# odecaux/DSP-Bench

Measured on AMD Instinct MI355X. Metric: Msamples/s offline render+8192-pt FFT, 48kHz stereo, 1/2/4/8 GPU; %HBM roofline, higher is better.
Workload: dtype f32

## Files before the change

dsp-bench_amd/csrc/stft_pk.hpp:

```cpp
#pragma once
#include "fft_pk.hpp"
#include "frame_load.hpp"

namespace dspb {

enum { kPkNoBarDft = 1, kPkNoBarTw = 2, kPkNoBarSplit = 4, kPkRenderCached = 8, kPkNtMag = 16, kPkMagLds = 32,
       kPkOldSplit = 64, kPkAbNoRender = 128, kPkAbNoMag = 256, kPkMagStage = 512, kPkOcc3 = 1024,
       kPkMemAos = 2048, kPkNoRemap = 4096, kPkAbNoXpose = 8192, kPkMemPf = 16384, kPkW1 = 65536,
       kPkMemHop = 131072, kPkNoReuse = 262144 };
constexpr int kPkDefaultOpt = kPkNoBarDft | kPkNoBarTw | kPkNoBarSplit;
constexpr int kPkPerOpt = kPkDefaultOpt | kPkW1;

typedef float f4u __attribute__((ext_vector_type(4), aligned(4)));
typedef float f4a __attribute__((ext_vector_type(4)));

template <bool NT, typename T>
__device__ __forceinline__ void st(T *p, T v) {
    if constexpr (NT) __builtin_nontemporal_store(v, p);
    else *p = v;
}

template <bool NT>
__device__ __forceinline__ void st4u(float *p, f4u v) {
    if constexpr (NT) __builtin_nontemporal_store(v, reinterpret_cast<f4u *>(p));
    else *reinterpret_cast<f4u *>(p) = v;
}

template <int KM>
__device__ __forceinline__ void put_bin(float *mrow, uint32_t K, uint32_t k, float m) {
    if constexpr (KM == kKPartial) {
        if (k < K) mrow[k] = m;
    } else {
        mrow[k] = m;
        if constexpr (KM == kKMirror) mrow[(8192u - k) & 8191u] = m;
    }
}

constexpr int kPkRowRegs = 66;
template <int KM, bool BAR, bool NOSTORE = false, bool STAGE = false, bool STAGE_NT = false, bool KEEP = false>
__device__ __forceinline__ void split_y2(const cx2 (&Y2)[32], float *mrow, uint32_t K, const v2f *tw,
                                         uint32_t lane, float *lds, float *M = nullptr) {
    static_assert(!STAGE || KM == kKHalf, "staged rows: 4097 bins");
    static_assert(!KEEP || (KM == kKHalf && !NOSTORE && !STAGE), "kept rows: 4097 bins, the dword row stores");
    float acc = 0.f;
    const uint32_t a = (uint32_t)(reinterpret_cast<uintptr_t>(mrow) >> 2) & 3u;
    float *sl = lds + a;
    const uint32_t src = ((64u - lane) & 63u) * 4u;
    const bool l0 = lane == 0;
    const v2f wl = tw[lane];
#pragma unroll
    for (int q = 0; q < 16; ++q) {
        if (BAR) __builtin_amdgcn_sched_barrier(0);
        const cx2 a = Y2[q == 0 ? 0 : 32 - q], b = Y2[31 - q];
        const float sxr = l0 ? (q == 0 ? a.r.x : a.r.y) : b.r.y;
        const float sxi = l0 ? (q == 0 ? a.i.x : a.i.y) : b.i.y;
        const float syr = l0 ? (q == 0 ? a.r.y : a.r.x) : b.r.x;
        const float syi = l0 ? (q == 0 ? a.i.y : a.i.x) : b.i.x;
        const cx2 Pp = cx2{v2f{bperm(src, sxr), bperm(src, syr)}, v2f{bperm(src, sxi), bperm(src, syi)}};
        const cx2 Z = Y2[q];
        const cx2 E = cx2{Z.r + Pp.r, Z.i - Pp.i};
        const cx2 D = cx2{Z.r - Pp.r, Z.i + Pp.i};
        v2f u = wl;
        if (q) u = v2f{wl.x, wl.x} * v2f{kW128_re[q], kW128_im[q]} + v2f{wl.y, wl.y} * v2f{-kW128_im[q], kW128_re[q]};
        v2f rU2, iU2;
        asm("v_pk_mul_f32 %0, %1, %2 op_sel:[0,1] op_sel_hi:[1,0] neg_hi:[0,1]" : "=v"(rU2) : "v"(D.r), "v"(u));
        asm("v_pk_mul_f32 %0, %1, %2 op_sel:[0,1] op_sel_hi:[1,0] neg_hi:[0,1]" : "=v"(iU2) : "v"(D.i), "v"(u));
        const cx2 T = cx2{D.i * u + rU2, iU2 - D.r * u};
        const cx2 X1 = E + T;
        const cx2 X2 = E - T;
        const v2f q1 = X1.r * X1.r + X1.i * X1.i;
        const v2f q2 = X2.r * X2.r + X2.i * X2.i;
        const uint32_t k = lane + 64u * (uint32_t)q;
        if constexpr (KEEP) {
            (M + lane)[64 * (4 * q)] = __builtin_amdgcn_sqrtf(q1.x);
            (M + lane)[64 * (4 * q + 1)] = __builtin_amdgcn_sqrtf(q1.y);
            (M + lane)[64 * (4 * q + 2)] = __builtin_amdgcn_sqrtf(q2.x);
            (M + lane)[64 * (4 * q + 3)] = __builtin_amdgcn_sqrtf(q2.y);
        } else if constexpr (NOSTORE) {
            acc += __builtin_amdgcn_sqrtf(q1.x) + __builtin_amdgcn_sqrtf(q1.y) + __builtin_amdgcn_sqrtf(q2.x) +
                   __builtin_amdgcn_sqrtf(q2.y);
        } else if constexpr (STAGE) {
            (sl + lane)[64 * q] = __builtin_amdgcn_sqrtf(q1.x);
            (sl + 2048u + lane)[64 * q] = __builtin_amdgcn_sqrtf(q1.y);
            (sl + 4096u - lane)[-64 * q] = __builtin_amdgcn_sqrtf(q2.x);
            (sl + 2048u - lane)[-64 * q] = __builtin_amdgcn_sqrtf(q2.y);
        } else if constexpr (KM == kKHalf) {
            st<STAGE_NT>(&(mrow + lane)[64 * q], __builtin_amdgcn_sqrtf(q1.x));
            st<STAGE_NT>(&(mrow + 2048u + lane)[64 * q], __builtin_amdgcn_sqrtf(q1.y));
            st<STAGE_NT>(&(mrow + 4096u - lane)[-64 * q], __builtin_amdgcn_sqrtf(q2.x));
            st<STAGE_NT>(&(mrow + 2048u - lane)[-64 * q], __builtin_amdgcn_sqrtf(q2.y));
        } else {
            put_bin<KM>(mrow, K, k, __builtin_amdgcn_sqrtf(q1.x));
            put_bin<KM>(mrow, K, 2048u + k, __builtin_amdgcn_sqrtf(q1.y));
            put_bin<KM>(mrow, K, 4096u - k, __builtin_amdgcn_sqrtf(q2.x));
            put_bin<KM>(mrow, K, 2048u - k, __builtin_amdgcn_sqrtf(q2.y));
        }
    }
    if constexpr (NOSTORE) {
        if (acc == -1.f) mrow[lane] = acc;
        return;
    }
    if (l0) {
        const cx z1 = cx{Y2[16].r.x, Y2[16].i.x}, z2 = cx{Y2[16].r.y, Y2[16].i.y};
        const cx E = cx{z1.r + z2.r, z1.i - z2.i}, D = cx{z1.r - z2.r, z1.i + z2.i};
        const float c = 0x1.6a09e6p-1f;
        const cx T = cx{c * (D.i - D.r), -c * (D.i + D.r)};
        const cx X1 = E + T, X2 = E - T;
        const float m1 = __builtin_amdgcn_sqrtf(__builtin_fmaf(X1.r, X1.r, X1.i * X1.i));
        const float m2 = __builtin_amdgcn_sqrtf(__builtin_fmaf(X2.r, X2.r, X2.i * X2.i));
        if constexpr (KEEP) {
            M[4096] = m1;
            M[4097] = m2;
        } else if constexpr (STAGE) {
            sl[1024] = m1;
            sl[3072] = m2;
        } else {
            put_bin<KM>(mrow, K, 1024u, m1);
            put_bin<KM>(mrow, K, 3072u, m2);
        }
    }
    if constexpr (STAGE) {
        lds_fence();
        const uint32_t j0 = a ? 1u : 0u, j1 = (4093u + a) >> 2;
        float *gb = mrow - a;
#pragma unroll
        for (int it = 0; it < 16; ++it) {
            const uint32_t j = j0 + 64u * (uint32_t)it + lane;
            if (it < 15 || j <= j1)
            {
                const float4 q = reinterpret_cast<const float4 *>(lds)[j];
                st<STAGE_NT>(reinterpret_cast<f4a *>(gb + 4u * j), f4a{q.x, q.y, q.z, q.w});
            }
        }
        const uint32_t head = 4u * j0 - a, tail0 = 4u * j1 + 4u - a;
        if (lane < head) mrow[lane] = sl[lane];
        if (lane >= 8u && tail0 + (lane - 8u) < 4097u) mrow[tail0 + lane - 8u] = sl[tail0 + lane - 8u];
    }
}

template <bool NT>
__device__ __forceinline__ void store_row_y2(const float (&M)[kPkRowRegs], float *mrow, uint32_t lane) {
#pragma unroll
    for (int q = 0; q < 16; ++q) {
        st<NT>(&(mrow + lane)[64 * q], M[4 * q]);
        st<NT>(&(mrow + 2048u + lane)[64 * q], M[4 * q + 1]);
        st<NT>(&(mrow + 4096u - lane)[-64 * q], M[4 * q + 2]);
        st<NT>(&(mrow + 2048u - lane)[-64 * q], M[4 * q + 3]);
    }
    if (lane == 0) {
        mrow[1024] = M[64];
        mrow[3072] = M[65];
    }
}

template <int OPT>
constexpr uint32_t pk_waves_per_block() { return (OPT & kPkW1) ? 1u : 4u; }
constexpr uint32_t kPkWpb = pk_waves_per_block<kPkDefaultOpt>();
constexpr uint32_t kPkPerWpb = pk_waves_per_block<kPkPerOpt>();

template <int PER>
__device__ __forceinline__ void per_gather(const Stft8kArgs &A, uint32_t p0, cx2 (&X)[PER >= 2 ? PER / 2 : 1]) {
    constexpr int NJ = PER >= 2 ? PER / 2 : 1;
    const float *T = A.map.table;
    if (A.map.closed) {
#pragma unroll
        for (int jj = 0; jj < NJ; ++jj) {
            const uint32_t q0 = (p0 + 256u * jj) & A.map.b_mask;
            const uint32_t q1 = (p0 + 256u * jj + (PER >= 2 ? 128u : 0u)) & A.map.b_mask;
            X[jj] = cx2{v2f{ramp_value(A.map, q0), ramp_value(A.map, q1)},
                        v2f{ramp_value(A.map, q0 + 1), ramp_value(A.map, q1 + 1)}};
        }
    } else {
#pragma unroll
        for (int jj = 0; jj < NJ; ++jj) {
            const uint32_t q0 = (p0 + 256u * jj) & A.map.b_mask;
            const uint32_t q1 = (p0 + 256u * jj + (PER >= 2 ? 128u : 0u)) & A.map.b_mask;
            X[jj] = cx2{v2f{T[q0], T[q1]}, v2f{T[q0 + 1], T[q1 + 1]}};
        }
    }
}

template <int PER, bool NT>
__device__ __forceinline__ void per_render_hop(const Stft8kArgs &A, float *o, uint32_t lane,
                                               const cx2 (&X)[PER >= 2 ? PER / 2 : 1]) {
    constexpr int NS = PER >= 2 ? PER : 1;
    v2f st[NS];
#pragma unroll
    for (int b = 0; b < NS; ++b) st[b] = v2f{X[b / 2].r[b & 1], X[b / 2].i[b & 1]};
    if (A.H == 4096u) {
#pragma unroll
        for (int b = 0; b < 32; ++b)
            dspb::st<NT>(reinterpret_cast<v2f *>(o + 128u * (uint32_t)b) + lane, st[b % NS]);
    } else {
#pragma unroll
        for (int b = 0; b < 64; ++b)
            if (128u * (uint32_t)b < A.H)
                dspb::st<NT>(reinterpret_cast<v2f *>(o + 128u * (uint32_t)b) + lane, st[b % NS]);
    }
}

template <int SRC, int KM, MapKind MK, bool POW2, bool WINC, int PER = 0, int OPT = kPkDefaultOpt, int OCC = 2>
__global__ __launch_bounds__(64 * pk_waves_per_block<OPT>()) __attribute__((amdgpu_waves_per_eu(OCC, OCC)))
void stft8192_pk_kernel(Stft8kArgs A) {
    constexpr uint32_t WPB = pk_waves_per_block<OPT>();
    __shared__ __attribute__((aligned(16))) float lds_all[WPB][OCC >= 3 ? 64 * 33 : 64 * 65];
    const uint32_t lane = threadIdx.x & 63u;
    const uint32_t wave = __builtin_amdgcn_readfirstlane(threadIdx.x >> 6);
    const uint32_t ch = blockIdx.y;
    uint64_t f = (uint64_t)((OPT & kPkNoRemap) ? blockIdx.x : xcd_remap(blockIdx.x, gridDim.x)) * WPB + wave;
    constexpr bool SOA = WINC && MK == MapKind::Ramp && PER > 0 && SRC == kSrcRender;
    constexpr bool REUSE = SOA && KM == kKHalf && OCC == 2 &&
                           !(OPT & (kPkNoReuse | kPkOldSplit | kPkMagLds | kPkMagStage | kPkAbNoRender | kPkAbNoMag | kPkAbNoXpose));
    uint32_t nrun = 1;
    if constexpr (REUSE) {
        if (A.run > 1u) {
            if (f < A.run_waves) {
                f *= A.run;
                const uint64_t left = A.F - f;
                nrun = left < A.run ? (uint32_t)left : A.run;
            } else {
                f = A.F + (f - A.run_waves);
            }
        }
    }
    constexpr bool MSOA = WINC && SRC == kSrcMemory && !(OPT & kPkMemAos);
    constexpr bool W4 = SOA && (8 % (PER >= 2 ? PER / 2 : 1)) == 0 && OCC == 2 &&
                        !(OPT & (kPkOldSplit | kPkMagLds | kPkAbNoXpose));
    const uint64_t fs = f * (uint64_t)A.H;
    if (f >= A.F) {
        if constexpr (SOA) {
            if (fs < A.tail_end) {
                const uint32_t p0 = (uint32_t)(A.goff + fs) + 2u * lane;
                float *o = A.out.p[ch] + fs;
                const uint64_t n = A.tail_end - fs;
#pragma unroll 4
                for (uint32_t b = 0; 128u * b < A.H; ++b) {
                    const uint32_t e = 128u * b + 2u * lane;
                    if (e < n) {
                        const uint32_t q = (p0 + 128u * b) & A.map.b_mask;
                        const v2f t = A.map.closed ? v2f{ramp_value(A.map, q), ramp_value(A.map, q + 1)}
                                                   : v2f{A.map.table[q], A.map.table[q + 1]};
                        reinterpret_cast<v2f *>(o + 128u * b)[lane] = t;
                    }
                }
            }
        }
        return;
    }
    float *lds = lds_all[wave];
    const float *x = (ch < A.in_ch) ? A.in.p[ch] : nullptr;

    static_assert(OCC == 2 || (SOA && !(OPT & (kPkOldSplit | kPkMagLds | kPkMagStage))),
                  "3 waves per SIMD: the PER path with split_y2");
    cx tlo[8];
    cx2 thp[4];
    if constexpr (OCC == 2) {
#pragma unroll
        for (int j = 1; j < 8; ++j) {
            const v2f a = (A.tw + 8192u + 64u * (uint32_t)(j - 1))[lane];
            tlo[j] = cx{a.x, a.y};
        }
        const float4 *tp4 = reinterpret_cast<const float4 *>(A.tw + 8192u + 896u);
#pragma unroll
        for (int h = 0; h < 4; ++h) {
            const float4 t = tp4[64u * (uint32_t)h + lane];
            thp[h] = cx2{v2f{t.x, t.y}, v2f{t.z, t.w}};
        }
    }
    float4 wbase = float4{0.f, 0.f, 0.f, 0.f};
    if constexpr (WINC) wbase = A.wbase[lane];

    cx2 P[32];
    if constexpr (SOA || MSOA) {
        constexpr int NJ = PER >= 2 ? PER / 2 : 1;
        cx2 X[NJ];
        if constexpr (SOA) {
            per_gather<PER>(A, (uint32_t)(A.goff + fs) + 2u * lane, X);
            if (!(OPT & kPkAbNoRender) && nrun == 1u)
                per_render_hop<PER, !(OPT & kPkRenderCached)>(A, A.out.p[ch] + fs, lane, X);
        }
        const float ue = A.wb * wbase.x, ve = A.wb * wbase.y, uo = A.wb * wbase.z, vo = A.wb * wbase.w;
        if constexpr (SOA) {
            cx2 XA[NJ], XU[NJ], XV[NJ];
            const float wa = W4 ? 4.f * A.wa : A.wa;
#pragma unroll
            for (int jj = 0; jj < NJ; ++jj) {
                XA[jj] = cx2{X[jj].r * v2f{wa, wa}, X[jj].i * v2f{wa, wa}};
                XU[jj] = cx2{X[jj].r * v2f{ue, ue}, X[jj].i * v2f{uo, uo}};
                XV[jj] = cx2{X[jj].r * v2f{ve, ve}, X[jj].i * v2f{vo, vo}};
            }
            auto fma2 = [](v2f a, v2f b, v2f c) { return __builtin_elementwise_fma(a, b, c); };
            if constexpr (W4) {
                auto Sv = [](int j) { return v2f{kWinB_s[2 * j], kWinB_s[2 * j + 1]}; };
                auto Cv = [](int j) { return v2f{kWinB_c[2 * j], kWinB_c[2 * j + 1]}; };
#pragma unroll
                for (int j0 = 0; j0 < 8; ++j0) {
                    const int jj = j0 % NJ;
                    const v2f s0 = Sv(j0), s1 = Sv(j0 + 8), s2 = Sv(j0 + 16), s3 = Sv(j0 + 24);
                    const v2f c0 = Cv(j0), c1 = Cv(j0 + 8), c2 = Cv(j0 + 16), c3 = Cv(j0 + 24);
                    const cx2 xa = XA[jj], xu = XU[jj], xv = XV[jj];
                    const v2f sA = (s0 + s1) + (s2 + s3), cA = (c0 + c1) + (c2 + c3);
                    P[j0] = cx2{fma2(-xu.r, cA, fma2(xv.r, sA, xa.r)), fma2(-xu.i, cA, fma2(xv.i, sA, xa.i))};
                    const v2f sC = (s0 - s1) + (s2 - s3), cC = (c0 - c1) + (c2 - c3);
                    P[j0 + 16] = cx2{fma2(-xu.r, cC, xv.r * sC), fma2(-xu.i, cC, xv.i * sC)};
                    const v2f sT = s0 - s2, cT = c0 - c2, sQ = s1 - s3, cQ = c1 - c3;
                    const cx2 t1 = cx2{fma2(-xu.r, cT, xv.r * sT), fma2(-xu.i, cT, xv.i * sT)};
                    const cx2 q = cx2{fma2(-xu.r, cQ, xv.r * sQ), fma2(-xu.i, cQ, xv.i * sQ)};
                    P[j0 + 8] = cx2{t1.r + q.i, t1.i - q.r};
                    P[j0 + 24] = cx2{t1.r - q.i, t1.i + q.r};
                }
            } else {
#pragma unroll
                for (int j = 0; j < 32; ++j) {
                    const v2f C = v2f{kWinB_c[2 * j], kWinB_c[2 * j + 1]}, S = v2f{kWinB_s[2 * j], kWinB_s[2 * j + 1]};
                    const int jj = j % NJ;
                    P[j] = cx2{fma2(-XU[jj].r, C, fma2(XV[jj].r, S, XA[jj].r)),
                               fma2(-XU[jj].i, C, fma2(XV[jj].i, S, XA[jj].i))};
                }
            }
        } else {
#pragma unroll
        for (int j = 0; j < 32; ++j) {
            const v2f C = v2f{kWinB_c[2 * j], kWinB_c[2 * j + 1]}, S = v2f{kWinB_s[2 * j], kWinB_s[2 * j + 1]};
            const v2f we = (v2f{ve, ve} * S + v2f{A.wa, A.wa}) - v2f{ue, ue} * C;
            const v2f wo = (v2f{vo, vo} * S + v2f{A.wa, A.wa}) - v2f{uo, uo} * C;
            const v2f a = reinterpret_cast<const v2f *>(x + fs + 256u * (uint32_t)j)[lane];
            const v2f b = reinterpret_cast<const v2f *>(x + fs + 256u * (uint32_t)j + 128u)[lane];
            const cx2 xj = cx2{v2f{a.x, b.x}, v2f{a.y, b.y}};
            P[j] = cx2{xj.r * we, xj.i * wo};
        }
        }
    } else {
    cx v[64];
    if constexpr (SRC == kSrcMemory) {
        if (A.valid >= 8192u) {
#pragma unroll
            for (int b = 0; b < 64; ++b) {
                const v2f t = reinterpret_cast<const v2f *>(x + fs + 128u * (uint32_t)b)[lane];
                v[b] = cx{t.x, t.y};
            }
        } else {
#pragma unroll
            for (int b = 0; b < 64; ++b) {
                const uint32_t s = 2u * lane + 128u * (uint32_t)b;
                v2f t = v2f{0.f, 0.f};
                if (s < A.valid) t = reinterpret_cast<const v2f *>(x + fs + 128u * (uint32_t)b)[lane];
                v[b] = cx{t.x, t.y};
            }
        }
    } else {
        if constexpr (MK == MapKind::Ramp && POW2) {
            if (A.map.B >= 4u && A.map.B <= 4096u) lds_table_frame(A, lds, fs, lane, v);
            else s_render_frame<MK, POW2>(A, x, fs, lane, v);
        } else if constexpr (MK == MapKind::GainTable && POW2) {
            if (A.map.B >= 4u && A.map.B <= 512u) reg_gain_table_frame(A, x, fs, lane, v, ch);
            else if (A.map.B >= 4u && A.map.B <= 4096u) lds_gain_table_frame(A, lds, x, fs, lane, v, ch);
            else s_render_frame<MK, POW2>(A, x, fs, lane, v, ch);
        } else {
            s_render_frame<MK, POW2>(A, x, fs, lane, v, ch);
        }
        float *o = A.out.p[ch] + fs;
        constexpr bool NT = !(OPT & kPkRenderCached);
        if (A.H == 4096u) {
#pragma unroll
            for (int b = 0; b < 32; ++b)
                st<NT>(reinterpret_cast<v2f *>(o + 128u * (uint32_t)b) + lane, v2f{v[b].r, v[b].i});
        } else {
#pragma unroll
            for (int b = 0; b < 64; ++b)
                if (128u * (uint32_t)b < A.H)
                    st<NT>(reinterpret_cast<v2f *>(o + 128u * (uint32_t)b) + lane, v2f{v[b].r, v[b].i});
        }
    }

    {
        const v2f uu = v2f{A.wb * wbase.x, A.wb * wbase.z}, vv = v2f{A.wb * wbase.y, A.wb * wbase.w};
#pragma unroll
        for (int j = 0; j < 32; ++j) {
            v2f w[2];
#pragma unroll
            for (int h = 0; h < 2; ++h) {
                const int b = 2 * j + h;
                if constexpr (WINC) {
                    w[h] = (vv * kWinB_s[b] + v2f{A.wa, A.wa}) - uu * kWinB_c[b];
                } else {
                    w[h] = (A.win2 + 64u * (uint32_t)b)[lane];
                }
            }
            P[j] = cx2{v2f{v[2 * j].r * w[0].x, v[2 * j + 1].r * w[1].x},
                       v2f{v[2 * j].i * w[0].y, v[2 * j + 1].i * w[1].y}};
        }
    }
    }

    if constexpr (!(OPT & (kPkOldSplit | kPkMagLds))) {
        cx2 Y2[32];
        if constexpr (OCC >= 3) fft4096_pk_y2_lo<!(OPT & kPkNoBarDft)>(P, lds, A.tw, lane, Y2);
        else fft4096_pk_y2<!(OPT & kPkNoBarDft), !(OPT & kPkNoBarTw), (OPT & kPkAbNoXpose) != 0, NoHook, W4>(
            P, lds, tlo, thp, lane, Y2);
        if constexpr (REUSE) {
            if (nrun > 1u) {
                static_assert(64 * 65 >= 4098, "the kept row fits the wave's LDS tile");
                split_y2<KM, !(OPT & kPkNoBarSplit), false, false, false, true>(Y2, nullptr, A.K, A.tw, lane, lds, lds);
                float M[kPkRowRegs];
#pragma unroll
                for (int j = 0; j < 64; ++j) M[j] = (lds + lane)[64 * j];
                M[64] = lds[4096];
                M[65] = lds[4097];
                cx2 X[PER >= 2 ? PER / 2 : 1];
                per_gather<PER>(A, (uint32_t)(A.goff + fs) + 2u * lane, X);
                float *o = A.out.p[ch] + fs;
                float *mrow = A.mag.p[ch] + f * A.ld;
                for (uint32_t r = 0; r < nrun; ++r, o += A.H, mrow += A.ld) {
                    per_render_hop<PER, !(OPT & kPkRenderCached)>(A, o, lane, X);
                    store_row_y2<(OPT & kPkNtMag) != 0>(M, mrow, lane);
                }
                return;
            }
        }
        split_y2<KM, !(OPT & kPkNoBarSplit), (OPT & kPkAbNoMag) != 0, KM == kKHalf && (OPT & kPkMagStage) != 0,
                 (OPT & kPkNtMag) != 0>(Y2, A.mag.p[ch] + f * A.ld, A.K, A.tw, lane, lds);
        return;
    }

    cx zp[32], zm[32];
    fft4096_pk<false, !(OPT & kPkNoBarDft), !(OPT & kPkNoBarTw)>(P, lds, tlo, thp, lane, zp, zm);

    float *mrow = A.mag.p[ch] + f * A.ld;
    const uint32_t src = ((64u - lane) & 63u) * 4u;
    const bool l0 = lane == 0;
    const v2f wl2 = A.tw[lane];
    const cx wl = cx{wl2.x, wl2.y};
#pragma unroll
    for (int ka = 0; ka < 16; ++ka) {
        if (!(OPT & kPkNoBarSplit)) __builtin_amdgcn_sched_barrier(0);
        const cx a0 = ka == 0 ? zp[0] : zm[32 - ka], b0 = zm[31 - ka];
        const cx a1 = zm[16 - ka], b1 = zm[15 - ka];
        const cx s0 = cx{l0 ? a0.r : b0.r, l0 ? a0.i : b0.i};
        const cx s1 = cx{l0 ? a1.r : b1.r, l0 ? a1.i : b1.i};
        const cx2 Pp = cx2{v2f{bperm(src, s0.r), bperm(src, s1.r)}, v2f{bperm(src, s0.i), bperm(src, s1.i)}};
        const cx2 Z = cx2{v2f{zp[ka].r, zp[ka + 16].r}, v2f{zp[ka].i, zp[ka + 16].i}};
        const cx2 E = cx2{Z.r + Pp.r, Z.i - Pp.i};
        const cx2 D = cx2{Z.r - Pp.r, Z.i + Pp.i};
        const cx2 tw = cmulb(wl, cx2{v2f{kW128_re[ka], kW128_re[ka + 16]},
                                     v2f{kW128_im[ka], kW128_im[ka + 16]}});
        const cx2 T = cmul2(negi(D), tw);
        const cx2 X1 = E + T;
        const cx2 X2 = E - T;
        const v2f q1 = X1.r * X1.r + X1.i * X1.i;
        const v2f q2 = X2.r * X2.r + X2.i * X2.i;
        const float m1[2] = {__builtin_amdgcn_sqrtf(q1.x), __builtin_amdgcn_sqrtf(q1.y)};
        const float m2[2] = {__builtin_amdgcn_sqrtf(q2.x), __builtin_amdgcn_sqrtf(q2.y)};
#pragma unroll
        for (int h = 0; h < 2; ++h) {
            const uint32_t kk = (uint32_t)(ka + 16 * h);
            const uint32_t k1 = lane + 64u * kk;
            const uint32_t k2 = 4096u - k1;
            if constexpr (KM == kKHalf && (OPT & kPkMagLds)) {
                lds[64u * kk + lane] = m1[h];
                lds[4096u - 64u * kk - lane] = m2[h];
            } else if constexpr (KM == kKPartial) {
                if (k1 < A.K) mrow[k1] = m1[h];
                if (k2 < A.K) mrow[k2] = m2[h];
            } else {
                st<(OPT & kPkNtMag) != 0>(mrow + 64u * kk + lane, m1[h]);
                st<(OPT & kPkNtMag) != 0>(mrow + 4096u - 64u * kk - lane, m2[h]);
                if constexpr (KM == kKMirror) {
                    mrow[k1 == 0 ? 0u : 8192u - k1] = m1[h];
                    (mrow + 4096u + 64u * kk)[lane] = m2[h];
                }
            }
        }
    }
    if constexpr (KM == kKHalf && (OPT & kPkMagLds)) {
        if (l0) {
            const cx Z = zm[0];
            lds[2048] = 2.f * __builtin_amdgcn_sqrtf(__builtin_fmaf(Z.r, Z.r, Z.i * Z.i));
        }
        lds_fence();
#pragma unroll
        for (int i = 0; i < 16; ++i) {
            const float4 q = reinterpret_cast<const float4 *>(lds)[64 * i + lane];
            st4u<(OPT & kPkNtMag) != 0>(mrow + 256u * (uint32_t)i + 4u * lane, f4u{q.x, q.y, q.z, q.w});
        }
        if (l0) mrow[4096] = lds[4096];
        return;
    }
    if (l0) {
        const cx Z = zm[0];
        const float m = 2.f * __builtin_amdgcn_sqrtf(__builtin_fmaf(Z.r, Z.r, Z.i * Z.i));
        if (KM != kKPartial || 2048u < A.K) mrow[2048] = m;
        if (KM == kKMirror) mrow[6144] = m;
    }
}

int launch_pk_paths(const Stft8kArgs &A, bool fused, int km, bool pow2, bool winc, dim3 grid, hipStream_t s);
bool stft_pk_ab_dispatch(const Stft8kArgs &A, uint32_t C, bool fused, int opt, dim3 grid, hipStream_t s, int *st);


}
```

Baseline: 670,300.

## Stage reused magnitude rows through LDS for aligned vector stores and render early

When a run of identical frames reuses one magnitude row, each row is now written to LDS, read back as aligned float4s and stored to global memory in 16-byte pieces, with the unaligned head and tail written as scalars. Before this, each lane did scattered scalar stores. The repeated render hops also move to the front, issued right after the gather instead of being interleaved with the row stores, so the X gather is not repeated. This aims to cut store transactions on the write-bound magnitude output, at the cost of extra LDS traffic and fences per row.

New measurement: 689,900 (median of 6 runs). 2.9% higher.

```diff
diff --git a/dsp-bench_amd/csrc/stft_pk.hpp b/dsp-bench_amd/csrc/stft_pk.hpp
--- a/dsp-bench_amd/csrc/stft_pk.hpp
+++ b/dsp-bench_amd/csrc/stft_pk.hpp
@@ -153,6 +153,51 @@
     }
 }
 
+template <bool NT>
+__device__ __forceinline__ void store_row_pieces(const float (&M)[kPkRowRegs], float *mrow, uint32_t lane, float *lds) {
+    const uint32_t a = (uint32_t)(reinterpret_cast<uintptr_t>(mrow) >> 2) & 3u;
+    float *sl = lds + a;
+#pragma unroll
+    for (int q = 0; q < 16; ++q) {
+        (sl + lane)[64 * q] = M[4 * q];
+        (sl + 2048u + lane)[64 * q] = M[4 * q + 1];
+        (sl + 4096u - lane)[-64 * q] = M[4 * q + 2];
+        (sl + 2048u - lane)[-64 * q] = M[4 * q + 3];
+    }
+    if (lane == 0) {
+        sl[1024] = M[64];
+        sl[3072] = M[65];
+    }
+    lds_fence();
+    const uint32_t j0 = a ? 1u : 0u, j1 = (4093u + a) >> 2;
+    float *gb = mrow - a;
+    float4 p[16];
+#pragma unroll
+    for (int it = 0; it < 16; ++it) {
+        const uint32_t j = j0 + 64u * (uint32_t)it + lane;
+        p[it] = reinterpret_cast<const float4 *>(lds)[j];
+    }
+    lds_fence();
+#pragma unroll
+    for (int it = 0; it < 16; ++it) {
+        const uint32_t j = j0 + 64u * (uint32_t)it + lane;
+        if (it < 15 || j <= j1)
+            st<NT>(reinterpret_cast<f4a *>(gb + 4u * j), f4a{p[it].x, p[it].y, p[it].z, p[it].w});
+    }
+    const uint32_t head = 4u * j0 - a, tail0 = 4u * j1 + 4u - a;
+    if (lane < head) mrow[lane] = M[0];
+    if (4096u - lane >= tail0) (mrow + 4096u - lane)[0] = M[2];
+}
+
+#ifndef DSPB_PK_RUN_ROWS
+#define DSPB_PK_RUN_ROWS 1
+#endif
+#ifndef DSPB_PK_RUN_RENDER_FIRST
+#define DSPB_PK_RUN_RENDER_FIRST 1
+#endif
+constexpr int kPkRunRows = DSPB_PK_RUN_ROWS;
+constexpr bool kPkRunRenderFirst = DSPB_PK_RUN_RENDER_FIRST != 0;
+
 template <int OPT>
 constexpr uint32_t pk_waves_per_block() { return (OPT & kPkW1) ? 1u : 4u; }
 constexpr uint32_t kPkWpb = pk_waves_per_block<kPkDefaultOpt>();
@@ -276,8 +321,14 @@
         cx2 X[NJ];
         if constexpr (SOA) {
             per_gather<PER>(A, (uint32_t)(A.goff + fs) + 2u * lane, X);
-            if (!(OPT & kPkAbNoRender) && nrun == 1u)
-                per_render_hop<PER, !(OPT & kPkRenderCached)>(A, A.out.p[ch] + fs, lane, X);
+            if constexpr (REUSE && kPkRunRenderFirst) {
+                float *o = A.out.p[ch] + fs;
+                for (uint32_t r = 0; r < nrun; ++r, o += A.H)
+                    per_render_hop<PER, !(OPT & kPkRenderCached)>(A, o, lane, X);
+            } else {
+                if (!(OPT & kPkAbNoRender) && nrun == 1u)
+                    per_render_hop<PER, !(OPT & kPkRenderCached)>(A, A.out.p[ch] + fs, lane, X);
+            }
         }
         const float ue = A.wb * wbase.x, ve = A.wb * wbase.y, uo = A.wb * wbase.z, vo = A.wb * wbase.w;
         if constexpr (SOA) {
@@ -407,13 +458,21 @@
                 for (int j = 0; j < 64; ++j) M[j] = (lds + lane)[64 * j];
                 M[64] = lds[4096];
                 M[65] = lds[4097];
-                cx2 X[PER >= 2 ? PER / 2 : 1];
-                per_gather<PER>(A, (uint32_t)(A.goff + fs) + 2u * lane, X);
-                float *o = A.out.p[ch] + fs;
+                auto store_row = [&](float *mrow) {
+                    if constexpr (kPkRunRows == 0) store_row_y2<(OPT & kPkNtMag) != 0>(M, mrow, lane);
+                    else store_row_pieces<kPkRunRows == 2 || (OPT & kPkNtMag) != 0>(M, mrow, lane, lds);
+                };
                 float *mrow = A.mag.p[ch] + f * A.ld;
-                for (uint32_t r = 0; r < nrun; ++r, o += A.H, mrow += A.ld) {
-                    per_render_hop<PER, !(OPT & kPkRenderCached)>(A, o, lane, X);
-                    store_row_y2<(OPT & kPkNtMag) != 0>(M, mrow, lane);
+                if constexpr (kPkRunRenderFirst) {
+                    for (uint32_t r = 0; r < nrun; ++r, mrow += A.ld) store_row(mrow);
+                } else {
+                    cx2 X[PER >= 2 ? PER / 2 : 1];
+                    per_gather<PER>(A, (uint32_t)(A.goff + fs) + 2u * lane, X);
+                    float *o = A.out.p[ch] + fs;
+                    for (uint32_t r = 0; r < nrun; ++r, o += A.H, mrow += A.ld) {
+                        per_render_hop<PER, !(OPT & kPkRenderCached)>(A, o, lane, X);
+                        store_row(mrow);
+                    }
                 }
                 return;
             }
```
